# Raiden-Makoto/MLX-VAE

Measured on AMD Instinct MI355X. Metric: SELFIES sequences/sec (whole node), AR-CVAE training step, higher is better.
Workload: dtype f32

## Files before the change

mlx-vae_amd/csrc/lstm.hip:

```cpp
#include "ops.h"
#include "skinny.h"
#include "xcd.h"

namespace {

__device__ __forceinline__ int xcd_group_block(int x, int gx, int on) {
    return (on && (gx & 7) == 0) ? (x & 7) * (gx >> 3) + (x >> 3) : x;
}

struct FwdJob {
    const float* xin;
    const float* Wx;
    const float* hprev;
    const float* Wh;
    const float* pre;
    const int32_t* tok;
    const float* cprev;
    float* h;
    float* ht;
    float* c;
    float* gates;
    void* oct;
};
struct FwdArgs {
// ... 1294 lines not shown
}

inline bool choose_step2(int B) {
    const int force = arcvae_env_int("ARCVAE_STEP_TILE", -1);
    if (force == 22) return true;
    if (force >= 0) return false;
    return B >= 256;
}


constexpr int PS_FLAGS = 0, PS_CNT = 256, PS_WORDS = 272;
constexpr int PS_BWD = 512;
constexpr int PS2_FWD_FLAGS = 1024, PS2_FWD_CNT = 1536, PS2_BWD_FLAGS = 1552, PS2_BWD_CNT = 2064, PS2_CU = 2304;
constexpr int PS2_WORDS = PS2_CU + 8 * 256;
constexpr int PS3_DONE = PS2_WORDS, PS3_WORDS = PS3_DONE + 512;
struct PersistArgs {
    const int32_t* x_tb;
    const float* table0;
    const float* bias[ARCVAE_MAX_LAYERS];
    const float* W[7];
    float* hseq;
    float* cseq;
    float* gseq;
    float* comb;
    unsigned* sync;
    unsigned* flags;
    unsigned* cnt;
    unsigned* cucnt;
    unsigned* start_signal;
    unsigned long long* trace;
    int B, T, H, V, RX, prio;
    int stagger;
};

__device__ __forceinline__ void ps_stagger(unsigned grp, int units) {
    if (grp != 0 && units > 0) {
        const unsigned long long t0 = wall_clock64();
        while (wall_clock64() - t0 < (unsigned long long)units) __builtin_amdgcn_s_sleep(8);
    }
}

typedef short s16x4_l __attribute__((ext_vector_type(4)));
typedef unsigned u32x2_l __attribute__((ext_vector_type(2)));
__device__ __forceinline__ s16x4_l pk4_bf16(f32x4 v) {
    const unsigned lo = __builtin_bit_cast(unsigned, __builtin_convertvector(f32x2_l{v.x, v.y}, bf16x2_l));
    const unsigned hi = __builtin_bit_cast(unsigned, __builtin_convertvector(f32x2_l{v.z, v.w}, bf16x2_l));
    return __builtin_bit_cast(s16x4_l, u32x2_l{lo, hi});
}

constexpr bool persist_wreg(int NT, int LL) { return (2 * LL - 1) * (2 * NT) * NT <= 32; }

#ifdef ARCVAE_PS_STAMPS
#define PS_STAMP(k) do { if (tr) a.trace[8 * (long)s + (k)] = wall_clock64(); } while (0)
#define PS_STAMP_START() PS_STAMP(1)
#define PS_STAMP_END() PS_STAMP(7)
#else
#define PS_STAMP(k) do { } while (0)
#define PS_STAMP_START() do { if (tr) a.trace[2 * s] = wall_clock64(); } while (0)
#define PS_STAMP_END() do { if (tr) a.trace[2 * s + 1] = wall_clock64(); } while (0)
#endif

template <int NG>
__device__ __forceinline__ void ps_take_role(unsigned* cnt, unsigned* cucnt, unsigned xcc, unsigned& grp, unsigned& role) {
    if constexpr (NG == 1) {
        grp = 0;
        role = atomicAdd(cnt + (xcc & 7), 1u);
    } else {
        unsigned g, r;
        if (cucnt) {
            unsigned hwid;
            asm volatile("s_getreg_b32 %0, hwreg(HW_REG_HW_ID)" : "=s"(hwid));
            g = atomicAdd(cucnt + (xcc & 7) * 256 + ((hwid >> 8) & 0xff), 1u) & 1u;
            r = atomicAdd(cnt + g * 8 + (xcc & 7), 1u);
            if (r >= 32) { g ^= 1u; r = atomicAdd(cnt + g * 8 + (xcc & 7), 1u); }
        } else {
            g = 0;
            r = atomicAdd(cnt + (xcc & 7), 1u);
            if (r >= 32) { g = 1; r = atomicAdd(cnt + 8 + (xcc & 7), 1u); }
        }
        grp = g; role = r;
    }
}

template <int NT, int LL, int RT, int MF = 0, int NG = 1>
__global__ __launch_bounds__(256, NG) void lstm_fwd_persist_kernel(PersistArgs a) {
    static_assert(MF == 0 || (NT == 2 && RT == 1 && LL <= 2), "4x4x1 form: H = 256, one row tile, L <= 2");
    static_assert(NG == 1 || (RT == 1 && MF == 0), "two groups: one 16-row tile per group");
    constexpr int CW = 16 * NT;
    constexpr int UW = 4 * NT;
    constexpr int NCH = 8 * NT;
    constexpr int CHW = NCH / 4;
    constexpr int S = 2 * LL - 1;
    constexpr int TPL = 256 / LL;
    constexpr int MAXP = (16 * RT * UW + TPL - 1) / TPL;
    constexpr bool WREG = (persist_wreg(NT, LL) && RT == 1) || MF;
    extern __shared__ __attribute__((aligned(16))) float lds[];
    float* wl = lds;
    float* red = WREG ? lds : lds + S * NCH * CW * 16;
    constexpr int RW = LL * 16 * RT * CW;
    __shared__ unsigned s_role, s_xcc, s_ok, s_grp;
    arcvae_set_prio(a.prio);
    const int tid = threadIdx.x, lane = tid & 63, wave = tid >> 6;
    const int B = a.B, T = a.T, H = a.H, G = 4 * a.H;
    if (tid == 0) {
        s_xcc = ps_xcc_id();
        unsigned g_, r_;
        ps_take_role<NG>(a.cnt, a.cucnt, s_xcc, g_, r_);
        s_grp = g_; s_role = r_;
        s_ok = 1;
        if (blockIdx.x == 0 && a.start_signal)
            __hip_atomic_fetch_add(a.start_signal, 1u, __ATOMIC_RELAXED, __HIP_MEMORY_SCOPE_AGENT);
    }
    __syncthreads();
    const unsigned xcc = __builtin_amdgcn_readfirstlane(s_xcc), role = __builtin_amdgcn_readfirstlane(s_role);
    const unsigned grp = NG == 1 ? 0u : __builtin_amdgcn_readfirstlane(s_grp);
    if (xcc >= 8 || role >= 32) {
        if (tid == 0) atomicAdd(a.sync + PS_ERR, 1u);
        return;
    }
    const int RX = NG == 1 ? a.RX : max(0, min(16, a.RX - 16 * (int)grp));
    const bool tr = a.trace && xcc == 0 && role == 0 && grp == 0 && tid == 0;
    auto wsrc = [&](int si, int kc, int rp, int ko) -> const float* {
        return a.W[si] + (long)(((rp >> 2) & 3) * H + (rp >> 4) * 4 + (rp & 3)) * H + 16 * kc + ko;
    };
    const int r = lane & 15, q4 = (lane >> 4) * 4;
    const int rg = lane >> 5, cg = (lane >> 2) & 7, ij = lane & 3;
    f32x4 wr[(WREG && !MF) ? S : 1][(WREG && !MF) ? CHW : 1][(WREG && !MF) ? NT : 1];
    f32x4 wq[MF == 1 ? S : 1][MF == 1 ? CHW : 1][MF == 1 ? 4 : 1];
    s16x4_l wqb[MF == 2 ? S : 1][MF == 2 ? CHW : 1][MF == 2 ? 4 : 1];
    {
        if constexpr (MF == 2) {
#pragma unroll
            for (int si = 0; si < S; ++si)
#pragma unroll
                for (int c = 0; c < CHW; ++c)
#pragma unroll
                    for (int g4 = 0; g4 < 4; ++g4)
                        wqb[si][c][g4] = pk4_bf16(*reinterpret_cast<const f32x4*>(wsrc(si, wave * CHW + c, role * CW + 4 * cg + ij, 4 * g4)));
        } else if constexpr (MF == 1) {
#pragma unroll
            for (int si = 0; si < S; ++si)
#pragma unroll
                for (int c = 0; c < CHW; ++c)
#pragma unroll
                    for (int g4 = 0; g4 < 4; ++g4)
                        wq[si][c][g4] = *reinterpret_cast<const f32x4*>(wsrc(si, wave * CHW + c, role * CW + 4 * cg + ij, 4 * g4));
        } else if constexpr (WREG) {
#pragma unroll
            for (int si = 0; si < S; ++si)
#pragma unroll
                for (int c = 0; c < CHW; ++c)
#pragma unroll
                    for (int n = 0; n < NT; ++n)
                        wr[si][c][n] = *reinterpret_cast<const f32x4*>(wsrc(si, wave * CHW + c, role * CW + 16 * n + r, q4));
        } else {
            for (int i = tid; i < S * NCH * CW * 4; i += 256) {
                const int si = i / (NCH * CW * 4), rem = i - si * (NCH * CW * 4);
                const int kc = rem / (CW * 4), c4 = rem - kc * (CW * 4);
                reinterpret_cast<float4*>(wl)[i] = *reinterpret_cast<const float4*>(wsrc(si, kc, role * CW + (c4 >> 2), (c4 & 3) * 4));
            }
        }
    }
    __syncthreads();
    const int row0 = xcc * a.RX + 16 * (int)grp;
    int arow[RT];
#pragma unroll
    for (int rt = 0; rt < RT; ++rt) arow[rt] = min(row0 + max(min(16 * rt + r, RX - 1), 0), B - 1);
    const int mrow = min(row0 + max(min(4 * rg + ij, RX - 1), 0), B - 1);
    const int el = min(tid / TPL, LL - 1), tl = tid - el * TPL;
    const bool eactive = tid < LL * TPL;
// ... 131 lines not shown
        }
        PS_STAMP(2);
#pragma unroll
        for (int l = 0; l < LL; ++l) {
            const int t = s - l;
            if (t < 0 || t >= T) continue;
            f32x4 acc[RT][NT];
#pragma unroll
            for (int rt = 0; rt < RT; ++rt)
#pragma unroll
                for (int n = 0; n < NT; ++n) acc[rt][n] = f32x4{0.f, 0.f, 0.f, 0.f};
#define PS_SRC(FR, SIDX)                                                                                         \
            _Pragma("unroll") for (int c = 0; c < CHW; ++c) {                                                    \
                const int kc = wave * CHW + c;                                                                   \
                _Pragma("unroll") for (int n = 0; n < NT; ++n) {                                                 \
                    f32x4 w;                                                                                      \
                    if constexpr (WREG) w = wr[WREG ? (SIDX) : 0][WREG ? c : 0][WREG ? n : 0];                     \
                    else w = *reinterpret_cast<const f32x4*>(wl + (((SIDX) * NCH + kc) * CW + 16 * n + r) * 16 + q4); \
                    _Pragma("unroll") for (int rt = 0; rt < RT; ++rt) {                                          \
                        acc[rt][n] = __builtin_amdgcn_mfma_f32_16x16x4f32(FR[l][rt][c].x, w.x, acc[rt][n], 0, 0, 0); \
                        acc[rt][n] = __builtin_amdgcn_mfma_f32_16x16x4f32(FR[l][rt][c].y, w.y, acc[rt][n], 0, 0, 0); \
                        acc[rt][n] = __builtin_amdgcn_mfma_f32_16x16x4f32(FR[l][rt][c].z, w.z, acc[rt][n], 0, 0, 0); \
                        acc[rt][n] = __builtin_amdgcn_mfma_f32_16x16x4f32(FR[l][rt][c].w, w.w, acc[rt][n], 0, 0, 0); \
                    }                                                                                            \
                }                                                                                                \
            }
            if (l > 0) { PS_SRC(fx, LL + l - 1) }
            if (t > 0) { PS_SRC(fh, l) }
#undef PS_SRC
            float* rp = red + wave * RW + l * 16 * RT * CW;
#pragma unroll
            for (int rt = 0; rt < RT; ++rt)
#pragma unroll
                for (int n = 0; n < NT; ++n)
#pragma unroll
                    for (int reg = 0; reg < 4; ++reg)
                        rp[(16 * rt + (lane >> 4) * 4 + reg) * CW + 16 * n + r] = acc[rt][n][reg];
        }
        }
        PS_STAMP(3);
        __syncthreads();
#ifndef ARCVAE_PS_STAMPS
        PS_STAMP(4);
#endif
        const int te = s - el;
        if (eactive && te >= 0 && te < T) {
#pragma unroll
            for (int i = 0; i < MAXP; ++i) {
                const int p = tl + i * TPL;
                if (p >= RX * UW) break;
                const int erow = p / UW, ul = p - erow * UW;
                const int b = row0 + erow;
                if (b >= B) continue;
                const int unit = role * UW + ul;
                const int cb = erow * CW + 16 * (ul >> 2) + (ul & 3);
                float v[4];
#pragma unroll
                for (int g = 0; g < 4; ++g) {
                    const int o = el * 16 * RT * CW + cb + 4 * g;
                    v[g] = (red[o] + red[RW + o]) + (red[2 * RW + o] + red[3 * RW + o]);
                }
                const float gi = chain_sigmoid(v[0] + pv[i][0]);
                const float gf = chain_sigmoid(v[1] + pv[i][1]);
                const float gg = chain_tanh(v[2] + pv[i][2]);
                const float go = chain_sigmoid(v[3] + pv[i][3]);
                const float c = te > 0 ? gf * cst[i] + gi * gg : gi * gg;
                cst[i] = c;
                const long hb = (long)b * H + unit;
                const float hval = go * chain_tanh(c);
                a.hseq[el * lH + (long)te * sH + hb] = hval;
                if (a.comb && el == LL - 1 && te == T - 1) a.comb[(long)b * 2 * H + unit] = hval;
                float* gp = a.gseq + el * lG + (long)te * sG + (long)b * G + unit;
                gp[0] = gi; gp[H] = gf; gp[2 * H] = gg; gp[3 * H] = go;
                a.cseq[el * lH + (long)te * sH + hb] = c;
            }
        }
        PS_STAMP(5);
        ps_stores_in_l2();
        PS_STAMP(6);
        __syncthreads();
        if (tid == 0) __hip_atomic_store(my_flag, (unsigned)(s + 1), __ATOMIC_RELAXED, __HIP_MEMORY_SCOPE_WORKGROUP);
        PS_STAMP_END();
    }
}

template <int NT, int LL, int RT, int MF = 0, int NG = 1>
void launch_persist(const PersistArgs& a, size_t lds, hipStream_t s) {
    (void)hipFuncSetAttribute((const void*)lstm_fwd_persist_kernel<NT, LL, RT, MF, NG>,
                              hipFuncAttributeMaxDynamicSharedMemorySize, 150 * 1024);
    hipLaunchKernelGGL((lstm_fwd_persist_kernel<NT, LL, RT, MF, NG>), dim3(256 * NG), dim3(256), lds, s, a);
}
inline size_t persist2_lds_bytes() {
    int kb = arcvae_env_int("ARCVAE_PERSIST2_LDS_KB", 56);
    kb = kb < 54 ? 54 : (kb > 80 ? 80 : kb);
    return (size_t)kb * 1024;
}
inline bool persist_two_groups(int B, int H, int L, int which ) {
    return (arcvae_env_int("ARCVAE_PERSIST2", 1) & which) != 0 && H == 256 && L >= 1 && L <= 2 && ceil_div(B, 8) > 16 && ceil_div(B, 8) <= 32;
}
inline int persist_row_tiles(int B) { return ceil_div(B, 8) > 16 ? 2 : 1; }
inline size_t persist_lds_floor() { return (size_t)arcvae_env_int("ARCVAE_PERSIST_LDS_KB", 81) * 1024; }
inline size_t persist_lds_bytes(int B, int H, int L) {
    const int NT = H / 128, CW = 16 * NT;
    const size_t red = sizeof(float) * (size_t)4 * L * 16 * persist_row_tiles(B) * CW;
    if (persist_wreg(NT, L) && persist_row_tiles(B) == 1)
        return red > persist_lds_floor() ? red : persist_lds_floor();
    return sizeof(float) * (size_t)(2 * L - 1) * (H / 16) * CW * 16 + red;
}
inline bool persist_shape_ok(int B, int T, int H, int L) {
    if (arcvae_env_int("ARCVAE_PERSIST", 1) == 0) return false;
    if (H % 128 != 0 || H / 128 > 3 || L < 1 || L > 4 || B < 1 || T < 1) return false;
    if (ceil_div(B, 8) > 32) return false;
    return persist_lds_bytes(B, H, L) <= 150 * 1024;
}


struct PersistBwdArgs {
    const float* wT;
    const float* cseq;
    const float* gseq;
    const float* dh_top;
    float* dG;
    float* dcs;
    float* dxs;
    unsigned* sync;
    unsigned* flags;
    unsigned* cnt;
    unsigned* cucnt;
    unsigned* err;
    unsigned* start_signal;
    unsigned long long* trace;
    int B, T, H, RX, RS, ld_dh_top, s_begin, s_end, cnt_off, prio;
    int stagger;
    int row_base, row_xs;
};

template <int NT, int LL, int RT>
__global__ __launch_bounds__(256) void lstm_bwd_persist_kernel(PersistBwdArgs a) {
    constexpr int UW = 4 * NT;
    constexpr int NCHB = 32 * NT;
    constexpr int CHB = NCHB / 4;
    constexpr int S = 2 * LL - 1;
    constexpr int NH = RT;
    constexpr int CHP = CHB / NH;
    constexpr int NP = 16 * RT * UW;
    constexpr int MAXP = (NP + 63) / 64;
    extern __shared__ __attribute__((aligned(16))) float lds[];
    float* wl = lds;
    float* red = wl + S * NCHB * UW * 16;
    float* dxl = red + 4 * S * 256 * RT;
    __shared__ unsigned s_role, s_xcc, s_ok;
    arcvae_set_prio(a.prio);
    const int tid = threadIdx.x, lane = tid & 63, wave = tid >> 6;
    const int B = a.B, T = a.T, H = a.H, G = 4 * a.H, RX = a.RX, RS = a.RS;
    if (tid == 0) {
        s_xcc = ps_xcc_id();
        s_role = atomicAdd(a.cnt + (s_xcc & 7), 1u);
        s_ok = 1;
        if (blockIdx.x == 0 && a.start_signal)
            __hip_atomic_fetch_add(a.start_signal, 1u, __ATOMIC_RELAXED, __HIP_MEMORY_SCOPE_AGENT);
    }
    __syncthreads();
    const unsigned xcc = __builtin_amdgcn_readfirstlane(s_xcc), role = __builtin_amdgcn_readfirstlane(s_role);
    if (xcc >= 8 || role >= 32) {
        if (tid == 0) atomicAdd(a.err, 1u);
        return;
    }
    const bool tr = a.trace && xcc == 0 && role == 0 && tid == 0;
    {
        const long wsz = (long)H * G;
        for (int i = tid; i < S * NCHB * UW * 4; i += 256) {
            const int sidx = i / (NCHB * UW * 4), rem = i - sidx * (NCHB * UW * 4);
            const int kc = rem / (UW * 4), c4 = rem - kc * (UW * 4);
            const int widx = sidx < LL ? (LL - 1 - sidx) : sidx;
            reinterpret_cast<float4*>(wl)[i] =
                *reinterpret_cast<const float4*>(a.wT + widx * wsz + ((long)kc * H + role * UW) * 16 + c4 * 4);
        }
    }
    __syncthreads();
    const int r = lane & 15, q4 = (lane >> 4) * 4;
    const int row0 = xcc * RX;
    int arow[RT];
#pragma unroll
// ... 771 lines not shown
    const bool step2 = !tile_mt && choose_step2(B);
    const int RS = operand_ring_slots(B, T, H, L, flags);
    for (int s = 0; s < T + L - 1; ++s) {
        FwdArgs a;
        a.B = B; a.H = H; a.V = V; a.prio = arcvae_step_prio(); a.remap = arcvae_xcd_remap() | (arcvae_env_int("ARCVAE_TILE_XCD", 0) != 0 ? 2 : 0); a.trace = trace ? trace + 2 * (long)s : nullptr;
        a.dbg = arcvae_env_int("ARCVAE_TILE_DEBUG", 0); a.lite = 0;
        int nj = 0;
        for (int l = 0; l < L; ++l) {
            const int t = s - l;
            if (t < 0 || t >= T) continue;
            FwdJob& j = a.job[nj++];
            j.xin = l > 0 ? hseq_t + ((long)(l - 1) * RS + (t % RS)) * sHt : nullptr;
            j.Wx = l > 0 ? wt + (L + l - 1) * wsz : nullptr;
            j.hprev = t > 0 ? hseq_t + ((long)l * RS + ((t - 1) % RS)) * sHt : nullptr;
            j.Wh = wt + l * wsz;
            j.pre = l > 0 ? bias[l] : table0;
            j.tok = l > 0 ? nullptr : x_tb + (long)t * B;
            j.cprev = t > 0 ? cseq + l * lH + (t - 1) * sH : nullptr;
            j.h = hseq + l * lH + t * sH;
            j.ht = hseq_t + ((long)l * RS + (t % RS)) * sHt;
            j.c = cseq + l * lH + t * sH;
            j.gates = gseq + l * lG + t * sG;
            j.oct = oct ? static_cast<char*>(h_oct) + 2 * (l * lH + t * sH) : nullptr;
        }
        for (int k = nj; k < ARCVAE_MAX_LAYERS; ++k) a.job[k] = a.job[0];
        if (tile_mt && s3) {
            if (tile_mt == 44) launch_fwd_tile<4, 4, 2>(a, B, H, nj, stream);
            else if (tile_mt == 4) launch_fwd_tile<4, 2, 2>(a, B, H, nj, stream);
            else if (tile_mt == 2) launch_fwd_tile<2, 2, 2>(a, B, H, nj, stream);
            else launch_fwd_tile<1, 2, 2>(a, B, H, nj, stream);
            continue;
        }
        if (tile_mt && b16) {
            if (tile_mt == 44) launch_fwd_tile<4, 4, 1>(a, B, H, nj, stream);
            else if (tile_mt == 4) launch_fwd_tile<4, 2, 1>(a, B, H, nj, stream);
            else if (tile_mt == 2) launch_fwd_tile<2, 2, 1>(a, B, H, nj, stream);
            else launch_fwd_tile<1, 2, 1>(a, B, H, nj, stream);
            continue;
        }
        if (tile_mt) {
            if (tile_mt == 44) launch_fwd_tile<4, 4>(a, B, H, nj, stream);
            else if (tile_mt == 4) launch_fwd_tile<4, 2>(a, B, H, nj, stream);
            else if (tile_mt == 2) launch_fwd_tile<2, 2>(a, B, H, nj, stream);
            else launch_fwd_tile<1, 2>(a, B, H, nj, stream);
            continue;
        }
        if (step2) {
            dim3 grid2(H / 8, ceil_div(B, 32), nj);
            DISPATCH_CH(H, launch_fwd2, a, grid2, stream)
            continue;
        }
        dim3 grid(H / 4, ceil_div(B, 16), nj);
        DISPATCH_CH(H, launch_fwd, a, grid, stream)
    }
    return arcvae_launch_status();
}


extern "C" int arcvae_enc_lstm_persistent_ok(int B, int T, int H, int L) { return persist_shape_ok(B, T, H, L) ? 1 : 0; }

extern "C" int arcvae_enc_lstm_forward_persistent(const int32_t* x_tb, const float* table0, const float* const* Wx,
                                                  const float* const* Wh, const float* const* bias, float* hseq,
                                                  float* cseq, float* gseq, float* wT_bwd, long wT_bwd_floats, float* comb,
                                                  unsigned* sync_ws, unsigned* start_signal, int B, int T, int V, int H,
                                                  int L, int flags, unsigned long long* trace, hipStream_t stream) {
    if (!x_tb || !table0 || !Wx || !Wh || !bias || !hseq || !cseq || !gseq || !sync_ws) return ARCVAE_ERR_ARG;
    if (V <= 0 || !persist_shape_ok(B, T, H, L)) return ARCVAE_ERR_ARG;
    if (wT_bwd) {
        long need[4];
        lstm_ws_need(B, T, H, L, flags, need);
        if (wT_bwd_floats < need[3]) return ARCVAE_ERR_ARG;
    }
    for (int l = 0; l < L; ++l)
        if (!Wh[l] || (l > 0 && (!Wx[l] || !bias[l]))) return ARCVAE_ERR_ARG;
    int rc;
    if (wT_bwd) {
        rc = tile_all_weights(Wx, Wh, nullptr, wT_bwd, H, L, 0,
                              bwd_split3(B, H, L, flags) ? 2 : (bwd_bf16(B, H, L, flags) ? 1 : 0), stream);
        if (rc != ARCVAE_OK) return rc;
    }
    if (!(flags & 1)) {
        rc = arcvae_zero(reinterpret_cast<float*>(sync_ws), 1, PS_WORDS, PS_WORDS, stream);
        if (rc != ARCVAE_OK) return rc;
    }
    PersistArgs a;
    a.x_tb = x_tb; a.table0 = table0; a.hseq = hseq; a.cseq = cseq; a.gseq = gseq; a.comb = comb;
    for (int i = 0; i < 7; ++i) a.W[i] = Wh[0];
    for (int l = 0; l < L; ++l) { a.W[l] = Wh[l]; if (l > 0) a.W[L + l - 1] = Wx[l]; }
    for (int l = 0; l < ARCVAE_MAX_LAYERS; ++l) a.bias[l] = (l > 0 && l < L) ? bias[l] : nullptr;
    a.sync = sync_ws; a.start_signal = start_signal; a.trace = trace;
    a.flags = sync_ws + PS_FLAGS; a.cnt = sync_ws + PS_CNT; a.cucnt = nullptr; a.stagger = 0;
    a.B = B; a.T = T; a.H = H; a.V = V; a.RX = ceil_div(B, 8); a.prio = arcvae_step_prio();
    if (persist_two_groups(B, H, L, 1)) {
        if (!(flags & 1)) {
            rc = arcvae_zero(reinterpret_cast<float*>(sync_ws + PS2_FWD_FLAGS), 1, PS2_WORDS - PS2_FWD_FLAGS, PS2_WORDS - PS2_FWD_FLAGS, stream);
            if (rc != ARCVAE_OK) return rc;
        }
        a.flags = sync_ws + PS2_FWD_FLAGS; a.cnt = sync_ws + PS2_FWD_CNT;
        a.stagger = arcvae_env_int("ARCVAE_PERSIST2_STAGGER_FWD", 200);
        a.cucnt = arcvae_env_int("ARCVAE_PERSIST2_ASSIGN", 1) != 0 ? sync_ws + PS2_CU : nullptr;
        if (L == 1) launch_persist<2, 1, 1, 0, 2>(a, persist2_lds_bytes(), stream);
        else launch_persist<2, 2, 1, 0, 2>(a, persist2_lds_bytes(), stream);
        return arcvae_launch_status();
    }
    const size_t lds = persist_lds_bytes(B, H, L);
    const int NT = H / 128;
    const int RTn = persist_row_tiles(B);
#define PS_LAUNCH(N_, L_) do { if (RTn == 2) launch_persist<N_, L_, 2>(a, lds, stream); else launch_persist<N_, L_, 1>(a, lds, stream); } while (0)
#define PS_BY_L(N_) switch (L) { case 1: PS_LAUNCH(N_, 1); break; case 2: PS_LAUNCH(N_, 2); break; case 3: PS_LAUNCH(N_, 3); break; default: PS_LAUNCH(N_, 4); break; }
    if (NT == 2 && L <= 2 && a.RX <= 8 && arcvae_env_int("ARCVAE_FWD_MFMA", 1) != 0) {
        if (flags & ARCVAE_PERSIST_BF16) {
            if (L == 1) launch_persist<2, 1, 1, 2>(a, lds, stream); else launch_persist<2, 2, 1, 2>(a, lds, stream);
        } else {
            if (L == 1) launch_persist<2, 1, 1, 1>(a, lds, stream); else launch_persist<2, 2, 1, 1>(a, lds, stream);
        }
    } else if (NT == 1) { PS_BY_L(1) } else if (NT == 2) { PS_BY_L(2) } else { PS_BY_L(3) }
#undef PS_BY_L
#undef PS_LAUNCH
    return arcvae_launch_status();
}


extern "C" int arcvae_enc_lstm_bwd_persistent_ok(int B, int T, int H, int L) { return persist_bwd_shape_ok(B, T, H, L) ? 1 : 0; }

extern "C" int arcvae_enc_lstm_backward_persistent(const float* cseq, const float* gseq, const float* dh_top,
                                                   int ld_dh_top, float* dG, float* dcs, float* dxs, const float* wT,
                                                   unsigned* sync_ws, unsigned* start_signal, int B, int T, int H,
                                                   int L, int s_begin, int s_end, int chunk_index,
                                                   unsigned long long* trace, hipStream_t stream) {
    if (!cseq || !gseq || !dh_top || !dG || !dcs || !dxs || !wT || !sync_ws) return ARCVAE_ERR_ARG;
    if (!persist_bwd_shape_ok(B, T, H, L) || ld_dh_top < H) return ARCVAE_ERR_ARG;
    const int S = T + 2 * (L - 1);
    if (s_begin < 0 || s_end > S || s_begin >= s_end) return ARCVAE_ERR_ARG;
    if (chunk_index < 0 || chunk_index >= 8 || (chunk_index == 0) != (s_begin == 0)) return ARCVAE_ERR_ARG;
    if (chunk_index == 0) {
        const int rc = arcvae_zero(reinterpret_cast<float*>(sync_ws + PS_BWD), 1, PS_WORDS + 64, PS_WORDS + 64, stream);
        if (rc != ARCVAE_OK) return rc;
    }
    PersistBwdArgs a;
    a.wT = wT; a.cseq = cseq; a.gseq = gseq; a.dh_top = dh_top; a.dG = dG; a.dcs = dcs; a.dxs = dxs;
    a.sync = sync_ws + PS_BWD; a.err = sync_ws + PS_ERR; a.start_signal = start_signal; a.trace = trace;
    a.B = B; a.T = T; a.H = H; a.RX = ceil_div(B, 8); a.RS = arcvae_ring_slots(T); a.ld_dh_top = ld_dh_top;
    a.row_base = 0; a.row_xs = a.RX;
    a.s_begin = s_begin; a.s_end = s_end; a.prio = arcvae_step_prio();
    a.cnt_off = chunk_index == 0 ? 0 : (PS_WORDS - PS_CNT) + 8 * (chunk_index - 1);
    a.flags = a.sync + PS_FLAGS; a.cnt = a.sync + PS_CNT + a.cnt_off; a.cucnt = nullptr; a.stagger = 0;
    const size_t lds = persist_bwd_lds_bytes(B, H, L);
    const int NT = H / 128;
    const int RTn = persist_row_tiles(B);
#define PB_BY_L(N_)                                                                                          \
    if (RTn == 2) { if (L == 1) launch_persist_bwd<N_, 1, 2>(a, lds, stream); else launch_persist_bwd<N_, 2, 2>(a, lds, stream); } \
    else { if (L == 1) launch_persist_bwd<N_, 1, 1>(a, lds, stream); else launch_persist_bwd<N_, 2, 1>(a, lds, stream); }
    if (NT == 1) { PB_BY_L(1) } else if (NT == 2) { PB_BY_L(2) } else { PB_BY_L(3) }
#undef PB_BY_L
    return arcvae_launch_status();
}


extern "C" int arcvae_enc_lstm_bwd_rs_halves(int B, int T, int H, int L) {
    return (arcvae_env_int("ARCVAE_PERSIST", 1) != 0 && arcvae_env_int("ARCVAE_RS_HALVES", 0) != 0 && H == 256 && L >= 1 && L <= 2 &&
            B > 128 && B <= 256 && T >= 1 && !persist_two_groups(B, H, L, 2)) ? 1 : 0;
}
extern "C" int arcvae_enc_lstm_bwd_rs_ok(int B, int T, int H, int L) {
    return (arcvae_env_int("ARCVAE_PERSIST", 1) != 0 && H == 256 && L >= 1 && L <= 2 && B >= 1 &&
            (B <= arcvae_env_int("ARCVAE_RS_MAX_B", 128) || persist_two_groups(B, H, L, 2) ||
             arcvae_enc_lstm_bwd_rs_halves(B, T, H, L) == 1) && B <= 256 && T >= 1) ? 1 : 0;
}

static inline long bwd_rs_part_floats(int B, int H, int L) {
    const int rows_x = ceil_div(B, 8);
    const int rgn = persist_two_groups(B, H, L, 2) ? 4 : (rows_x <= 8 ? 1 : (rows_x <= 16 ? 2 : 4));
    return (long)rgn * 2 * (2 * L - 1) * 8 * 32 * 32 * 64;
}
extern "C" long arcvae_enc_lstm_bwd_rs_part_floats(int B, int T, int H, int L) {
    return arcvae_enc_lstm_bwd_rs_ok(B, T, H, L) == 1 ? bwd_rs_part_floats(B, H, L) : 0;
}

extern "C" int arcvae_enc_lstm_persist_groups(int B, int H, int L) {
    return (arcvae_env_int("ARCVAE_PERSIST", 1) != 0 && B > 0 && persist_two_groups(B, H, L, 3)) ? 2 : 1;
}

namespace {
struct FusedWgrad {
    const float* hseq; const int32_t* x_tb; float* const* dWx; float* const* dWh; float* const* dbias; float* dtable; int V;
};
int launch_bwd_rs(const float* const* Wx, const float* const* Wh, const float* cseq, const float* gseq,
                  const float* dh_top, int ld_dh_top, float* dG, float* dcs, float* dxs, float* part_ws, long part_ws_floats,
                  unsigned* sync_ws, unsigned* start_signal, int B, int T, int H, int L, int s_begin, int s_end,
                  int chunk_index, unsigned long long* trace, const FusedWgrad* fused, int flags, hipStream_t stream) {
    if (!Wx || !Wh || !cseq || !gseq || !dh_top || !dG || !dcs || !dxs || !part_ws || !sync_ws) return ARCVAE_ERR_ARG;
    if (H != 256 || L < 1 || L > 2 || B < 1 || B > 256 || T < 1 || ld_dh_top < H) return ARCVAE_ERR_ARG;
    if (arcvae_env_int("ARCVAE_PERSIST", 1) == 0) return ARCVAE_ERR_ARG;
    if (part_ws_floats < bwd_rs_part_floats(B, H, L)) return ARCVAE_ERR_ARG;
    const bool halves = (flags & ARCVAE_RS_HALF) != 0;
    const int half = (flags & ARCVAE_RS_HALF1) ? 1 : 0;
// ... 533 lines not shown
```

Before: 66290.

## Split two-layer persistent LSTM forward into per-layer wave groups in one block

Adds a layer-split variant of the persistent fp32 MFMA LSTM forward kernel for H=256, L=2 and small batch. Each block runs 512 threads: one half computes layer 0 and the other layer 1. Layer 0 also computes layer 1's input projection and passes it through an LDS ring buffer, so the two layers advance in a pipelined, wavefront fashion instead of running sequentially per step. It uses separate global flag sets per layer and LDS counters for intra-block handoff. The cost is more threads and LDS per block plus more complex spin-wait synchronisation, which could stall or raise register pressure.

```diff
diff --git a/mlx-vae_amd/csrc/lstm.hip b/mlx-vae_amd/csrc/lstm.hip
--- a/mlx-vae_amd/csrc/lstm.hip
+++ b/mlx-vae_amd/csrc/lstm.hip
@@ -1400,10 +1400,241 @@
     }
 }
 
-template <int NT, int LL, int RT, int MF = 0, int NG = 1>
-__global__ __launch_bounds__(256, NG) void lstm_fwd_persist_kernel(PersistArgs a) {
+constexpr int PS_LS_FLAGS = 1024;
+constexpr int PS_LS_RD = 2;
+constexpr size_t PS_LS_LDS = sizeof(float) * (8192 + 2 * 1024 + PS_LS_RD * 4096) + 64 * sizeof(unsigned);
+
+__device__ __forceinline__ unsigned ls_ld(const unsigned* w) { return __hip_atomic_load(w, __ATOMIC_ACQUIRE, __HIP_MEMORY_SCOPE_WORKGROUP); }
+__device__ __forceinline__ void ls_st(unsigned* w, unsigned v) { __hip_atomic_store(w, v, __ATOMIC_RELEASE, __HIP_MEMORY_SCOPE_WORKGROUP); }
+
+__device__ void lstm_fwd_persist_split(const PersistArgs& a) {
+    constexpr int H = 256, G = 4 * H, CW = 32, UW = 8, CHW = 4, RD = PS_LS_RD;
+    extern __shared__ __attribute__((aligned(16))) float lds[];
+    f32x4* wxl = reinterpret_cast<f32x4*>(lds);
+    float* red = lds + 8192;
+    f32x4* ring = reinterpret_cast<f32x4*>(lds + 8192 + 2 * 1024);
+    unsigned* cw = reinterpret_cast<unsigned*>(lds + 8192 + 2 * 1024 + RD * 4096);
+    __shared__ unsigned s_role, s_xcc;
+    __shared__ int s_ok;
+    arcvae_set_prio(a.prio);
+    const int tid = threadIdx.x, lane = tid & 63, wave = tid >> 6, ly = wave >> 2, kw = wave & 3;
+    const int B = a.B, T = a.T;
+    if (tid == 0) {
+        s_xcc = ps_xcc_id();
+        unsigned g_, r_;
+        ps_take_role<1>(a.cnt, a.cucnt, s_xcc, g_, r_);
+        s_role = r_;
+        s_ok = 1;
+        if (blockIdx.x == 0 && a.start_signal)
+            __hip_atomic_fetch_add(a.start_signal, 1u, __ATOMIC_RELAXED, __HIP_MEMORY_SCOPE_AGENT);
+    }
+    if (tid < 16) cw[tid] = 0;
+    __syncthreads();
+    const unsigned xcc = __builtin_amdgcn_readfirstlane(s_xcc), role = __builtin_amdgcn_readfirstlane(s_role);
+    if (xcc >= 8 || role >= 32) {
+        if (tid == 0) atomicAdd(a.sync + PS_ERR, 1u);
+        return;
+    }
+    const int RX = a.RX, row0 = xcc * RX;
+    auto wsrc = [&](int si, int kc, int rp, int ko) -> const float* {
+        return a.W[si] + (long)(((rp >> 2) & 3) * H + (rp >> 4) * 4 + (rp & 3)) * H + 16 * kc + ko;
+    };
+    const int rg = lane >> 5, cg = (lane >> 2) & 7, ij = lane & 3;
+    f32x4 wq[CHW][4];
+#pragma unroll
+    for (int c = 0; c < CHW; ++c)
+#pragma unroll
+        for (int g4 = 0; g4 < 4; ++g4)
+            wq[c][g4] = *reinterpret_cast<const f32x4*>(wsrc(ly, kw * CHW + c, role * CW + 4 * cg + ij, 4 * g4));
+    for (int i = tid; i < 4 * CHW * 4 * 32; i += 512) {
+        const int l32 = i & 31, g4 = (i >> 5) & 3, kc = i >> 7;
+        wxl[i] = *reinterpret_cast<const f32x4*>(wsrc(2, kc, role * CW + 4 * (l32 >> 2) + (l32 & 3), 4 * g4));
+    }
+    __syncthreads();
+    const int mrow = min(row0 + max(min(4 * rg + ij, RX - 1), 0), B - 1);
+    const unsigned qoff = (unsigned)(((long)mrow * H + 64 * kw + 4 * cg) * 4);
+    const long sH = (long)B * H, sG = (long)B * G, lH = (long)T * sH, lG = (long)T * sG;
+    const unsigned* xflags = a.sync + (ly == 0 ? PS_FLAGS : PS_LS_FLAGS) + xcc * 32;
+    unsigned* my_flag = a.sync + (ly == 0 ? PS_FLAGS : PS_LS_FLAGS) + xcc * 32 + role;
+    const int erow = lane >> 3, ul = lane & 7, eb = row0 + erow, unit = role * UW + ul;
+    const bool eact = kw == 0 && erow < RX && eb < B;
+    const bool tr = a.trace && xcc == 0 && role == 0 && kw == 0 && lane == 0;
+#ifdef ARCVAE_PS_STAMPS
+#define LS_STAMP(k) do { if (tr) a.trace[8 * (long)t + 4 * ly + (k)] = wall_clock64(); } while (0)
+#else
+#define LS_STAMP(k) do { } while (0)
+#endif
+    auto lds_wait = [&](const unsigned* w, unsigned target) -> bool {
+        unsigned spins = 0;
+        while ((int)(ls_ld(w) - target) < 0) {
+            if (!__hip_atomic_load(&s_ok, __ATOMIC_RELAXED, __HIP_MEMORY_SCOPE_WORKGROUP) || ++spins > 4000000u) {
+                if (lane == 0) { atomicAdd(a.sync + PS_ERR, 1u); __hip_atomic_store(&s_ok, 0, __ATOMIC_RELAXED, __HIP_MEMORY_SCOPE_WORKGROUP); }
+                return false;
+            }
+            __builtin_amdgcn_s_sleep(1);
+        }
+        return true;
+    };
+    auto flags_seen = [&](int t) -> bool {
+        if (kw == 1) {
+            unsigned spins = 0;
+            while (true) {
+                const unsigned v = (lane < 32) ? __hip_atomic_load(xflags + lane, __ATOMIC_RELAXED, __HIP_MEMORY_SCOPE_AGENT) : (unsigned)t;
+                if (__all((int)(v - (unsigned)t) >= 0)) break;
+                if (++spins > 4000000u || __hip_atomic_load(a.sync + PS_ERR, __ATOMIC_RELAXED, __HIP_MEMORY_SCOPE_AGENT)
+                    || !__hip_atomic_load(&s_ok, __ATOMIC_RELAXED, __HIP_MEMORY_SCOPE_WORKGROUP)) {
+                    if (lane == 0) { atomicAdd(a.sync + PS_ERR, 1u); __hip_atomic_store(&s_ok, 0, __ATOMIC_RELAXED, __HIP_MEMORY_SCOPE_WORKGROUP); }
+                    return false;
+                }
+                __builtin_amdgcn_s_sleep(1);
+            }
+            if (lane == 0) ls_st(cw + ly, (unsigned)t);
+            return true;
+        }
+        return lds_wait(cw + ly, (unsigned)t);
+    };
+#define LS_Q1(Q, W_, M_, AB_)                                                                                                \
+    { const f32x4 w_ = W_(2 * M_ + (AB_ >> 2), AB_ & 3);                                                                   \
+      acc[0] = __builtin_amdgcn_mfma_f32_4x4x1f32(Q[M_].x, w_.x, acc[0], 3, AB_, 0);                                      \
+      acc[1] = __builtin_amdgcn_mfma_f32_4x4x1f32(Q[M_].y, w_.y, acc[1], 3, AB_, 0);                                      \
+      acc[2] = __builtin_amdgcn_mfma_f32_4x4x1f32(Q[M_].z, w_.z, acc[2], 3, AB_, 0);                                      \
+      acc[3] = __builtin_amdgcn_mfma_f32_4x4x1f32(Q[M_].w, w_.w, acc[3], 3, AB_, 0); }
+#define LS_Q8(Q, W_, M_) LS_Q1(Q, W_, M_, 0) LS_Q1(Q, W_, M_, 1) LS_Q1(Q, W_, M_, 2) LS_Q1(Q, W_, M_, 3) \
+                         LS_Q1(Q, W_, M_, 4) LS_Q1(Q, W_, M_, 5) LS_Q1(Q, W_, M_, 6) LS_Q1(Q, W_, M_, 7)
+#define LS_WREG(C_, G_) wq[C_][G_]
+#define LS_WLDS(C_, G_) wxl[((kw * CHW + (C_)) * 4 + (G_)) * 32 + (lane & 31)]
+    float cst = 0.f;
+    auto epilogue = [&](int t, const float (&pv)[4]) {
+        if (eact) {
+            const int cb = erow * CW + 16 * (ul >> 2) + (ul & 3);
+            const float* rl = red + ly * 1024;
+            float v[4];
+#pragma unroll
+            for (int g = 0; g < 4; ++g) {
+                const int o = cb + 4 * g;
+                v[g] = (rl[o] + rl[256 + o]) + (rl[512 + o] + rl[768 + o]);
+            }
+            const float gi = chain_sigmoid(v[0] + pv[0]);
+            const float gf = chain_sigmoid(v[1] + pv[1]);
+            const float gg = chain_tanh(v[2] + pv[2]);
+            const float go = chain_sigmoid(v[3] + pv[3]);
+            const float c = t > 0 ? gf * cst + gi * gg : gi * gg;
+            cst = c;
+            const long hb = (long)eb * H + unit;
+            const float hval = go * chain_tanh(c);
+            a.hseq[ly * lH + (long)t * sH + hb] = hval;
+            if (a.comb && ly == 1 && t == T - 1) a.comb[(long)eb * 2 * H + unit] = hval;
+            float* gp = a.gseq + ly * lG + (long)t * sG + (long)eb * G + unit;
+            gp[0] = gi; gp[H] = gf; gp[2 * H] = gg; gp[3 * H] = go;
+            a.cseq[ly * lH + (long)t * sH + hb] = c;
+        }
+        ps_stores_in_l2();
+        if (lane == 0) __hip_atomic_store(my_flag, (unsigned)(t + 1), __ATOMIC_RELAXED, __HIP_MEMORY_SCOPE_WORKGROUP);
+    };
+    auto put_partial = [&](const f32x4 (&acc)[4]) {
+        float* rp = red + ly * 1024 + kw * 256 + (4 * rg) * CW + 4 * cg + ij;
+#pragma unroll
+        for (int i = 0; i < 4; ++i) rp[i * CW] = (acc[0][i] + acc[1][i]) + (acc[2][i] + acc[3][i]);
+        if (lane == 0) __hip_atomic_fetch_add(cw + 2 + ly, 1u, __ATOMIC_RELEASE, __HIP_MEMORY_SCOPE_WORKGROUP);
+    };
+
+    if (ly == 0) {
+        for (int t = 0; t <= T; ++t) {
+            LS_STAMP(0);
+            float pv[4] = {0.f, 0.f, 0.f, 0.f};
+            if (eact && t < T) {
+                int tk = a.x_tb[(long)t * B + eb];
+                tk = min(max(tk, 0), a.V - 1);
+                const float* pre = a.table0 + (long)tk * G;
+                pv[0] = pre[unit]; pv[1] = pre[H + unit]; pv[2] = pre[2 * H + unit]; pv[3] = pre[3 * H + unit];
+            }
+#ifndef ARCVAE_PS_STAMPS
+            if (tr && t < T) a.trace[2 * t] = wall_clock64();
+#endif
+            if (t > 0 && !flags_seen(t)) return;
+            LS_STAMP(1);
+            f32x4 qh[2];
+            if (t > 0) {
+                const __amdgpu_buffer_rsrc_t rs = ps_rsrc(a.hseq + (long)(t - 1) * sH, sH * 4);
+                qh[0] = ps_load_sc1_x4(rs, qoff);
+                qh[1] = ps_load_sc1_x4(rs, qoff + 128);
+            }
+            if (t < T) {
+                f32x4 acc[4];
+#pragma unroll
+                for (int e = 0; e < 4; ++e) acc[e] = f32x4{0.f, 0.f, 0.f, 0.f};
+                if (t > 0) { LS_Q8(qh, LS_WREG, 0) LS_Q8(qh, LS_WREG, 1) }
+                put_partial(acc);
+                if (kw == 0) {
+                    if (!lds_wait(cw + 2, 4u * (unsigned)(t + 1))) return;
+                    LS_STAMP(2);
+                    epilogue(t, pv);
+                    LS_STAMP(3);
+#ifndef ARCVAE_PS_STAMPS
+                    if (tr && t == 0) a.trace[1] = wall_clock64();
+#endif
+                }
+            }
+            if (t > 0) {
+                const int j = t - 1;
+                if (j >= RD && !lds_wait(cw + 8 + kw, (unsigned)(j - RD + 1))) return;
+                f32x4 acc[4];
+#pragma unroll
+                for (int e = 0; e < 4; ++e) acc[e] = f32x4{0.f, 0.f, 0.f, 0.f};
+                LS_Q8(qh, LS_WLDS, 0) LS_Q8(qh, LS_WLDS, 1)
+                f32x4* rs = ring + ((j % RD) * 4 + kw) * 256 + lane;
+#pragma unroll
+                for (int e = 0; e < 4; ++e) rs[64 * e] = acc[e];
+                if (lane == 0) ls_st(cw + 4 + kw, (unsigned)(j + 1));
+            }
+        }
+    } else {
+        float pv[4] = {0.f, 0.f, 0.f, 0.f};
+        if (eact) { const float* pre = a.bias[1]; pv[0] = pre[unit]; pv[1] = pre[H + unit]; pv[2] = pre[2 * H + unit]; pv[3] = pre[3 * H + unit]; }
+        for (int t = 0; t < T; ++t) {
+            LS_STAMP(0);
+            if (t > 0 && !flags_seen(t)) return;
+            LS_STAMP(1);
+            f32x4 qh[2];
+            if (t > 0) {
+                const __amdgpu_buffer_rsrc_t rs = ps_rsrc(a.hseq + lH + (long)(t - 1) * sH, sH * 4);
+                qh[0] = ps_load_sc1_x4(rs, qoff);
+                qh[1] = ps_load_sc1_x4(rs, qoff + 128);
+            }
+            if (!lds_wait(cw + 4 + kw, (unsigned)(t + 1))) return;
+            f32x4 acc[4];
+            const f32x4* rs = ring + ((t % RD) * 4 + kw) * 256 + lane;
+#pragma unroll
+            for (int e = 0; e < 4; ++e) acc[e] = rs[64 * e];
+            if (t > 0) { LS_Q8(qh, LS_WREG, 0) LS_Q8(qh, LS_WREG, 1) }
+            put_partial(acc);
+            if (lane == 0) ls_st(cw + 8 + kw, (unsigned)(t + 1));
+            if (kw == 0) {
+                if (!lds_wait(cw + 3, 4u * (unsigned)(t + 1))) return;
+                LS_STAMP(2);
+                epilogue(t, pv);
+                LS_STAMP(3);
+#ifndef ARCVAE_PS_STAMPS
+                if (tr) a.trace[2 * (t + 1) + 1] = wall_clock64();
+#endif
+            }
+        }
+    }
+#undef LS_WLDS
+#undef LS_WREG
+#undef LS_Q8
+#undef LS_Q1
+#undef LS_STAMP
+}
+
+template <int NT, int LL, int RT, int MF = 0, int NG = 1, int LS = 0>
+__global__ __launch_bounds__(256 * (1 + LS), NG) void lstm_fwd_persist_kernel(PersistArgs a) {
     static_assert(MF == 0 || (NT == 2 && RT == 1 && LL <= 2), "4x4x1 form: H = 256, one row tile, L <= 2");
     static_assert(NG == 1 || (RT == 1 && MF == 0), "two groups: one 16-row tile per group");
+    static_assert(LS == 0 || (NT == 2 && LL == 2 && RT == 1 && MF == 1 && NG == 1), "layer split: H 256, L 2, fp32 4x4x1 form");
+    if constexpr (LS != 0) {
+        lstm_fwd_persist_split(a);
+    } else {
     constexpr int CW = 16 * NT;
     constexpr int UW = 4 * NT;
     constexpr int NCH = 8 * NT;
@@ -1701,13 +1932,14 @@
         if (tid == 0) __hip_atomic_store(my_flag, (unsigned)(s + 1), __ATOMIC_RELAXED, __HIP_MEMORY_SCOPE_WORKGROUP);
         PS_STAMP_END();
     }
-}
-
-template <int NT, int LL, int RT, int MF = 0, int NG = 1>
+    }
+}
+
+template <int NT, int LL, int RT, int MF = 0, int NG = 1, int LS = 0>
 void launch_persist(const PersistArgs& a, size_t lds, hipStream_t s) {
-    (void)hipFuncSetAttribute((const void*)lstm_fwd_persist_kernel<NT, LL, RT, MF, NG>,
+    (void)hipFuncSetAttribute((const void*)lstm_fwd_persist_kernel<NT, LL, RT, MF, NG, LS>,
                               hipFuncAttributeMaxDynamicSharedMemorySize, 150 * 1024);
-    hipLaunchKernelGGL((lstm_fwd_persist_kernel<NT, LL, RT, MF, NG>), dim3(256 * NG), dim3(256), lds, s, a);
+    hipLaunchKernelGGL((lstm_fwd_persist_kernel<NT, LL, RT, MF, NG, LS>), dim3(256 * NG), dim3(256 * (1 + LS)), lds, s, a);
 }
 inline size_t persist2_lds_bytes() {
     int kb = arcvae_env_int("ARCVAE_PERSIST2_LDS_KB", 56);
@@ -1718,6 +1950,10 @@
     return (arcvae_env_int("ARCVAE_PERSIST2", 1) & which) != 0 && H == 256 && L >= 1 && L <= 2 && ceil_div(B, 8) > 16 && ceil_div(B, 8) <= 32;
 }
 inline int persist_row_tiles(int B) { return ceil_div(B, 8) > 16 ? 2 : 1; }
+inline bool persist_layer_split(int B, int H, int L) {
+    return arcvae_env_int("ARCVAE_LAYER_SPLIT", 1) != 0 && arcvae_env_int("ARCVAE_FWD_MFMA", 1) != 0 && H == 256 && L == 2
+           && ceil_div(B, 8) <= 8;
+}
 inline size_t persist_lds_floor() { return (size_t)arcvae_env_int("ARCVAE_PERSIST_LDS_KB", 81) * 1024; }
 inline size_t persist_lds_bytes(int B, int H, int L) {
     const int NT = H / 128, CW = 16 * NT;
@@ -2655,6 +2891,10 @@
     if (!(flags & 1)) {
         rc = arcvae_zero(reinterpret_cast<float*>(sync_ws), 1, PS_WORDS, PS_WORDS, stream);
         if (rc != ARCVAE_OK) return rc;
+        if (!(flags & ARCVAE_PERSIST_BF16) && persist_layer_split(B, H, L)) {
+            rc = arcvae_zero(reinterpret_cast<float*>(sync_ws + PS_LS_FLAGS), 1, 256, 256, stream);
+            if (rc != ARCVAE_OK) return rc;
+        }
     }
     PersistArgs a;
     a.x_tb = x_tb; a.table0 = table0; a.hseq = hseq; a.cseq = cseq; a.gseq = gseq; a.comb = comb;
@@ -2684,6 +2924,8 @@
     if (NT == 2 && L <= 2 && a.RX <= 8 && arcvae_env_int("ARCVAE_FWD_MFMA", 1) != 0) {
         if (flags & ARCVAE_PERSIST_BF16) {
             if (L == 1) launch_persist<2, 1, 1, 2>(a, lds, stream); else launch_persist<2, 2, 1, 2>(a, lds, stream);
+        } else if (persist_layer_split(B, H, L)) {
+            launch_persist<2, 2, 1, 1, 1, 1>(a, lds > PS_LS_LDS ? lds : PS_LS_LDS, stream);
         } else {
             if (L == 1) launch_persist<2, 1, 1, 1>(a, lds, stream); else launch_persist<2, 2, 1, 1>(a, lds, stream);
         }
```

New measurement: 69110, median of 6. 1.04x the previous value.
